# pavlidic/Binary-SpGEMM

Hardware: AMD Instinct MI355X
Metric: output nnz/sec (GNZ/s) (higher is better)
Workload: dtype int32; 1 GPU; R-MAT scale 22, edge factor 16, (a,b,c,d)=(0.30,0.25,0.25,0.20), seed 1, A*A; n=4194304, nnz_a=67108664, products=1336443900, nnz_c=1336366087, parallelism=row-shards x1 cut at equal work, B replicated, priming_steps=0, flow=auto, full=False

## Files before the change

### binary-spgemm_amd/csrc/context.hip

```cpp
#include "internal.hpp"

using namespace bsp;

thread_local char bspgemm_err_text[512] = "";

extern "C" const char *bspgemm_last_error(void) { return g_err; }

extern "C" const char *bspgemm_status_string(bspgemm_status s)
{
    switch (s) {
    case BSPGEMM_OK: return "ok";
    case BSPGEMM_ERR_INVALID: return "invalid argument";
    case BSPGEMM_ERR_ALLOC: return "allocation failed";
    case BSPGEMM_ERR_HIP: return "HIP runtime error";
    case BSPGEMM_ERR_NO_DEVICE: return "no gfx950 device (this library has no CPU fallback)";
    case BSPGEMM_ERR_OVERFLOW: return "result exceeds the int32 drop-in interface";
    case BSPGEMM_ERR_IO: return "file I/O error";
    case BSPGEMM_ERR_FORMAT: return "Matrix Market banner rejected";
    case BSPGEMM_ERR_SIZE: return "Matrix Market size line or entry rejected";
    case BSPGEMM_ERR_COMM: return "RCCL error";
    }
    return "unknown status";
}

// ... 99 lines not shown
    HIPCHK(hipGetDeviceProperties(&prop, device));
    if (strncmp(prop.gcnArchName, "gfx950", 6) != 0) {
        snprintf(g_err, sizeof g_err, "device %d is %s; libbspgemm carries gfx950 code only", device,
                 prop.gcnArchName);
        return BSPGEMM_ERR_NO_DEVICE;
    }
    bspgemm_context *ctx = new (std::nothrow) bspgemm_context();
    if (!ctx) return FAIL(BSPGEMM_ERR_ALLOC, "context");
    auto bail = [&](bspgemm_status st) { bspgemm_destroy(ctx); return st; };
    ctx->device = device;
    HIPCHK_B(hipSetDevice(device));
    HIPCHK_B(hipStreamCreateWithFlags(&ctx->stream, hipStreamNonBlocking));
    ctx->own_stream = true;
    HIPCHK_B(hipHostMalloc(reinterpret_cast<void **>(&ctx->h), sizeof(HostScalars), hipHostMallocDefault));
    HIPCHK_B(hipMalloc(reinterpret_cast<void **>(&ctx->d_prep), sizeof(PrepScalars)));
    HIPCHK_B(hipMalloc(reinterpret_cast<void **>(&ctx->d_small), sizeof(SmallScalars)));
    HIPCHK_B(hipMalloc(reinterpret_cast<void **>(&ctx->d_small_tiles), sizeof(SmallTiles)));
    HIPCHK_B(hipMalloc(reinterpret_cast<void **>(&ctx->d_err), 64));
    HIPCHK_B(hipMemset(ctx->d_err, 0, 64));
    HIPCHK_B(hipMalloc(reinterpret_cast<void **>(&ctx->bin_count), kNumBins * sizeof(int)));
    for (auto &sl : ctx->slots) {
        for (auto &e : sl.ev) HIPCHK_B(hipEventCreate(&e));
        for (auto &ph : sl.ev_cls) for (auto &c : ph) for (auto &e : c) HIPCHK_B(hipEventCreate(&e));
    }
    HIPCHK_B(hipStreamCreateWithFlags(&ctx->stream_b, hipStreamNonBlocking));
    HIPCHK_B(hipStreamCreateWithFlags(&ctx->stream_c, hipStreamNonBlocking));
    HIPCHK_B(hipEventCreateWithFlags(&ctx->ev_join, hipEventDisableTiming));
    for (auto &t : ctx->ev_tile) for (auto &e : t) HIPCHK_B(hipEventCreateWithFlags(&e, hipEventDisableTiming));
    ctx->cache_budget = prop.totalGlobalMem / 4;
    if (const char *e = getenv("BSPGEMM_FLOW"))
        ctx->flow = !strcmp(e, "exact") ? BSPGEMM_FLOW_EXACT : (!strcmp(e, "upper-bound") || !strcmp(e, "ub")) ? BSPGEMM_FLOW_UPPER_BOUND : BSPGEMM_FLOW_AUTO;
    if (const char *e = getenv("BSPGEMM_CLASS_TIMING")) ctx->class_timing = atoi(e) != 0;
    if (const char *e = getenv("BSPGEMM_CLASS_STREAMS")) { const int n = atoi(e); ctx->class_streams = n < 1 ? 1 : (n > 3 ? 3 : n); }
    ctx->check = getenv("BSPGEMM_CHECK") != nullptr;
    if (const char *e = getenv("BSPGEMM_RW_BLK")) ctx->rw_blk = atoi(e) ? 1 : 0;
    if (const char *e = getenv("BSPGEMM_SMALL")) ctx->small = atoi(e) ? 1 : 0;
    if (const char *e = getenv("BSPGEMM_PAD_ROWS")) { const int v = atoi(e); ctx->pad_rows = v < 0 ? -1 : (v ? 1 : 0); }
    ctx->debug_alloc = getenv("BSPGEMM_DEBUG_ALLOC") != nullptr;
    ctx->dropin_timing = getenv("BSPGEMM_DROPIN_TIMING") != nullptr;
    if (ctx->debug_alloc)
        fprintf(stderr, "[bspgemm] device %d: %s, %zu MiB, %d CUs; result cache budget %zu MiB\n", device,
                prop.gcnArchName, (size_t)(prop.totalGlobalMem >> 20), prop.multiProcessorCount, ctx->cache_budget >> 20);
    *out = ctx;
    return BSPGEMM_OK;
}

extern "C" void bspgemm_destroy(bspgemm_context *ctx)
{
    if (!ctx) return;
    hipSetDevice(ctx->device);
    if (ctx->stream) hipStreamSynchronize(ctx->stream);
    hipFree(ctx->F); hipFree(ctx->Fprefix); hipFree(ctx->partials);
    hipFree(ctx->cnt); hipFree(ctx->bin_tiles); hipFree(ctx->bin_count); hipFree(ctx->tmp); hipFree(ctx->tmpv);
    hipFree(ctx->rec); hipFree(ctx->recpre); hipFree(ctx->ab); hipFree(ctx->Fmask); hipFree(ctx->hpartials);
    hipFree(ctx->hub_rec); hipFree(ctx->hub_pre);
    if (ctx->h) hipHostFree(ctx->h);
    hipFree(ctx->d_prep);
    hipFree(ctx->d_err);
    hipFree(ctx->d_small);
    hipFree(ctx->d_small_tiles);
    hipFree(ctx->chunk_row);
    for (auto &sl : ctx->slots) {
        for (auto &e : sl.ev) if (e) hipEventDestroy(e);
        for (auto &ph : sl.ev_cls) for (auto &c : ph) for (auto &e : c) if (e) hipEventDestroy(e);
    }
    for (auto &c : ctx->cache) if (c.p) hipFree(c.p);
    if (ctx->stream_b) { hipStreamSynchronize(ctx->stream_b); hipStreamDestroy(ctx->stream_b); }
    if (ctx->stream_c) { hipStreamSynchronize(ctx->stream_c); hipStreamDestroy(ctx->stream_c); }
    if (ctx->ev_join) hipEventDestroy(ctx->ev_join);
    hipFree(ctx->stitch_partials);
    for (auto &t : ctx->ev_tile) for (auto &e : t) if (e) hipEventDestroy(e);
    if (ctx->own_stream && ctx->stream) hipStreamDestroy(ctx->stream);
    delete ctx;
}

extern "C" bspgemm_status bspgemm_set_stream(bspgemm_context *ctx, void *hip_stream)
{
    if (!ctx) return FAIL(BSPGEMM_ERR_INVALID, "ctx is NULL");
    if (bspgemm_status st = use_device(ctx)) return st;
    HIPCHK(hipStreamSynchronize(ctx->stream));
    if (hip_stream) {
        if (ctx->own_stream) hipStreamDestroy(ctx->stream);
        ctx->stream = static_cast<hipStream_t>(hip_stream);
        ctx->own_stream = false;
    } else if (!ctx->own_stream) {
        HIPCHK(hipStreamCreateWithFlags(&ctx->stream, hipStreamNonBlocking));
        ctx->own_stream = true;
    }
    return BSPGEMM_OK;
}

extern "C" bspgemm_status bspgemm_synchronize(bspgemm_context *ctx)
{
    if (!ctx) return FAIL(BSPGEMM_ERR_INVALID, "ctx is NULL");
    if (bspgemm_status st = use_device(ctx)) return st;
    HIPCHK(hipStreamSynchronize(ctx->stream));
    return BSPGEMM_OK;
}

extern "C" bspgemm_status bspgemm_matrix_upload(bspgemm_context *ctx, int rows, int cols,
                                                const int *row_ptr, const int *col_idx,
                                                bspgemm_matrix **out)
{
    if (!ctx || !out || !row_ptr || rows < 0 || cols < 0) return FAIL(BSPGEMM_ERR_INVALID, "matrix_upload");
    *out = nullptr;
    const long long base = row_ptr[0];
    const long long nnz = (long long)row_ptr[rows] - base;
// ... 74 lines not shown
    m->nnz_pad = 0;
    return BSPGEMM_OK;
}

extern "C" const char *bspgemm_build_info(void)
{
    return "libbspgemm: HIP kernels for gfx950 only; flows upper-bound (default), exact; small-product path; "
           "timing-only ablation switches: none (BSP_ABLATE=0); tuning constants are compile-time";
}

extern "C" int bspgemm_matrix_rows(const bspgemm_matrix *m) { return m ? m->rows : 0; }
extern "C" int bspgemm_matrix_cols(const bspgemm_matrix *m) { return m ? m->cols : 0; }
extern "C" int64_t bspgemm_matrix_nnz(const bspgemm_matrix *m) { return m ? m->nnz : 0; }

bspgemm_status ensure_rows(bspgemm_context *ctx, size_t rows)
{
    if (rows <= ctx->rows_cap) return BSPGEMM_OK;
    HIPCHK(hipStreamSynchronize(ctx->stream));
    hipFree(ctx->F); hipFree(ctx->Fprefix); hipFree(ctx->partials); hipFree(ctx->cnt); hipFree(ctx->bin_tiles);
    hipFree(ctx->rec); hipFree(ctx->recpre); hipFree(ctx->Fmask); hipFree(ctx->hpartials);
    ctx->F = ctx->Fprefix = ctx->partials = ctx->recpre = ctx->Fmask = ctx->hpartials = nullptr;
    ctx->cnt = ctx->bin_tiles = nullptr;
    ctx->rec = nullptr;
    ctx->rows_cap = 0;
    const size_t cap = rows + rows / 8 + 64;
    const size_t tiles = cap / 2048 + 2;
    HIPCHK(hipMalloc(reinterpret_cast<void **>(&ctx->F), cap * sizeof(long long)));
    HIPCHK(hipMalloc(reinterpret_cast<void **>(&ctx->Fmask), cap * sizeof(long long)));
    HIPCHK(hipMalloc(reinterpret_cast<void **>(&ctx->Fprefix), (cap + 1) * sizeof(long long)));
    HIPCHK(hipMalloc(reinterpret_cast<void **>(&ctx->partials), (tiles + 1) * sizeof(long long)));
    HIPCHK(hipMalloc(reinterpret_cast<void **>(&ctx->hpartials), (tiles + 1) * sizeof(long long)));
    HIPCHK(hipMalloc(reinterpret_cast<void **>(&ctx->cnt), cap * sizeof(int)));
    HIPCHK(hipMalloc(reinterpret_cast<void **>(&ctx->bin_tiles), (tiles + 1) * kNumBins * sizeof(int)));
    HIPCHK(hipMalloc(reinterpret_cast<void **>(&ctx->rec), cap * sizeof(RowRec)));
    HIPCHK(hipMalloc(reinterpret_cast<void **>(&ctx->recpre), cap * sizeof(long long)));
    if (!ctx->hub_rec) {
        HIPCHK(hipMalloc(reinterpret_cast<void **>(&ctx->hub_rec), kHeavySortMax * sizeof(RowRec)));
        HIPCHK(hipMalloc(reinterpret_cast<void **>(&ctx->hub_pre), kHeavySortMax * sizeof(long long)));
    }
    ctx->rows_cap = cap;
    return BSPGEMM_OK;
}

bspgemm_status ensure_ab(bspgemm_context *ctx, size_t pairs)
{
    if (pairs <= ctx->ab_cap) return BSPGEMM_OK;
    HIPCHK(hipStreamSynchronize(ctx->stream));
    hipFree(ctx->ab);
    ctx->ab = nullptr;
    ctx->ab_cap = 0;
    const size_t cap = pairs + pairs / 16 + 64;
    HIPCHK(hipMalloc(reinterpret_cast<void **>(&ctx->ab), cap * sizeof(int2)));
    ctx->ab_cap = cap;
    return BSPGEMM_OK;
}

bspgemm_status ensure_tmp(bspgemm_context *ctx, size_t ints)
{
    if (ints <= ctx->tmp_cap) return BSPGEMM_OK;
    HIPCHK(hipStreamSynchronize(ctx->stream));
    hipFree(ctx->tmp);
    ctx->tmp = nullptr;
    ctx->tmp_cap = 0;
    const size_t cap = ints + ints / 16 + 1024;
    hipError_t e = hipMalloc(reinterpret_cast<void **>(&ctx->tmp), cap * sizeof(int));
    if (e == hipErrorOutOfMemory) {
        for (auto &c : ctx->cache) if (c.p) { hipFree(c.p); c.p = nullptr; }
        (void)hipGetLastError();
        e = hipMalloc(reinterpret_cast<void **>(&ctx->tmp), cap * sizeof(int));
    }
    HIPCHK(e);
    ctx->tmp_cap = cap;
    return BSPGEMM_OK;
}

bspgemm_status ensure_tmpv(bspgemm_context *ctx, size_t ints)
{
    if (ints <= ctx->tmpv_cap) return BSPGEMM_OK;
    HIPCHK(hipStreamSynchronize(ctx->stream));
    hipFree(ctx->tmpv);
    ctx->tmpv = nullptr;
    ctx->tmpv_cap = 0;
    const size_t cap = ints + ints / 16 + 1024;
    hipError_t e = hipMalloc(reinterpret_cast<void **>(&ctx->tmpv), cap * sizeof(int));
    if (e == hipErrorOutOfMemory) {
        for (auto &c : ctx->cache) if (c.p) { hipFree(c.p); c.p = nullptr; }
        (void)hipGetLastError();
        e = hipMalloc(reinterpret_cast<void **>(&ctx->tmpv), cap * sizeof(int));
    }
    HIPCHK(e);
    ctx->tmpv_cap = cap;
    return BSPGEMM_OK;
}

bspgemm_status ensure_chunk_rows(bspgemm_context *ctx, size_t entries)
{
    if (entries <= ctx->chunk_cap) return BSPGEMM_OK;
    HIPCHK(hipStreamSynchronize(ctx->stream));
    hipFree(ctx->chunk_row);
    ctx->chunk_row = nullptr;
    ctx->chunk_cap = 0;
    const size_t cap = entries + entries / 16 + 64;
    HIPCHK(hipMalloc(reinterpret_cast<void **>(&ctx->chunk_row), cap * sizeof(int)));
    ctx->chunk_cap = cap;
    return BSPGEMM_OK;
}
// ... 234 lines not shown
```

### binary-spgemm_amd/csrc/internal.hpp

```cpp
#pragma once
#include "../../include/bspgemm.h"
#include "kernels.hpp"

#include <hip/hip_runtime.h>

#include <climits>
#include <cstdio>
#include <cstdlib>
#include <cstring>
#include <chrono>
#include <new>

extern thread_local char bspgemm_err_text[512];
#define g_err bspgemm_err_text

static inline bspgemm_status fail(bspgemm_status st, const char *what, const char *file, int line)
{
    snprintf(g_err, sizeof g_err, "%s (%s:%d)", what, file, line);
    return st;
}
#define FAIL(st, what) fail((st), (what), __FILE__, __LINE__)
#define HIPCHK(call)                                                                       \
    do {                                                                                   \
        hipError_t e_ = (call);                                                            \
// ... 13 lines not shown
        }                                                                                  \
    } while (0)

using bsp::kNumBins;
using bsp::PrepScalars;
using bsp::RowRec;
struct HostScalars {
    long long totalF;
    long long nnzC;
    int bin_count[kNumBins];
    int a_lo, a_hi;
    long long products;
    long long heavy_total;
    PrepScalars prep;
    unsigned err;
    bsp::SmallScalars small;
};

struct bspgemm_context {
    int device = 0;
    hipStream_t stream = nullptr;
    bool own_stream = false;
    hipStream_t stream_b = nullptr;
    hipStream_t stream_c = nullptr;
    hipEvent_t ev_tile[2][3] = {};
    hipEvent_t ev_join = nullptr;
    struct StatSlot {
        hipEvent_t ev[5] = {};
        hipEvent_t ev_cls[2][kNumBins][2] = {};
        int R = 0;
        bool cls_timed = false;
        int mid_cap = 0, rank_cap = 0;
        HostScalars h = {};
        long long products = 0, nnz_c = 0;
        int cls_n[2][kNumBins] = {};
        bool used = false;
        int flow = 0, prepass_kernel = 0, class_streams = 0;
        bool small = false, checked = false, padded = false;
    };
    static constexpr int kStatSlots = 16;
    StatSlot slots[kStatSlots];
    int slot_head = 0;
    long long *stitch_partials = nullptr;
    size_t stitch_partials_cap = 0;
    size_t rows_cap = 0;
    long long *F = nullptr, *Fprefix = nullptr, *partials = nullptr, *recpre = nullptr, *Fmask = nullptr;
    long long *hpartials = nullptr;
    RowRec *hub_rec = nullptr;
    long long *hub_pre = nullptr;
    int *cnt = nullptr, *bin_tiles = nullptr, *bin_count = nullptr;
    RowRec *rec = nullptr;
    size_t ab_cap = 0;
    int2 *ab = nullptr;
    size_t tmp_cap = 0;
    int *tmp = nullptr;
    size_t tmpv_cap = 0;
    int *tmpv = nullptr;
    PrepScalars *d_prep = nullptr;
    bsp::SmallScalars *d_small = nullptr;
    bsp::SmallTiles *d_small_tiles = nullptr;
    unsigned *d_err = nullptr;
    int *chunk_row = nullptr;
    size_t chunk_cap = 0;
    HostScalars *h = nullptr;
    struct CachedBuf { void *p; size_t bytes; };
    CachedBuf cache[8] = {};
    size_t cache_budget = 0;
    int flow = BSPGEMM_FLOW_AUTO;
    bool class_timing = false;
    int class_streams = 2;
    bool check = false;
    int rw_blk = -1;
    int pad_rows = 0;
    int small = -1;
    bool debug_alloc = false;
    bool dropin_timing = false;
};

extern "C" int bspgemm_par_max_plus_one(const int *idx, long long n);
extern "C" void bspgemm_par_prefault(void *p, size_t bytes);
extern "C" long long bspgemm_par_output_bound(const int *Acol, const int *Arow, int r0, int r1, const int *Brow, int brows, long long cap);

struct bspgemm_matrix {
    bspgemm_context *ctx;
    int rows, cols;
    long long nnz;
    int *d_row_ptr, *d_col_idx;
    bool owned;
    mutable unsigned char *d_deg8 = nullptr;
    mutable int *d_blk8 = nullptr;
    mutable int blk8_state = 0;
    mutable int *d_col_pad = nullptr;
    mutable int *d_row_ptr_pad = nullptr;
    mutable int2 *d_ext = nullptr;
    mutable int pad_state = 0;
    mutable long long nnz_pad = 0;
    const int *gather_col() const { return pad_state == 1 ? d_col_pad : d_col_idx; }
    long long gather_nnz() const { return pad_state == 1 ? nnz_pad : nnz; }
};

bspgemm_status ensure_deg8(const bspgemm_matrix *m);
bspgemm_status ensure_blk8(const bspgemm_matrix *m);
bspgemm_status ensure_pad(const bspgemm_matrix *m);

struct bspgemm_result {
    bspgemm_context *ctx;
    int rows;
    long long nnz;
    long long *d_row_ptr;
    int *d_col_idx;
    long long col_cap;
    int *d_values = nullptr;
};

bspgemm_status use_device(bspgemm_context *ctx);

bspgemm_status ensure_rows(bspgemm_context *ctx, size_t rows);
bspgemm_status ensure_ab(bspgemm_context *ctx, size_t pairs);
bspgemm_status ensure_tmp(bspgemm_context *ctx, size_t ints);
bspgemm_status ensure_tmpv(bspgemm_context *ctx, size_t ints);
bspgemm_status ensure_chunk_rows(bspgemm_context *ctx, size_t entries);
bool result_cached(const bspgemm_context *ctx, size_t bytes);
hipError_t result_alloc(bspgemm_context *ctx, void **out, size_t bytes);
void result_release(bspgemm_context *ctx, void *p, size_t bytes);
static inline size_t result_bytes_rowptr(int rows) { return ((size_t)rows + 1) * sizeof(long long); }
static inline size_t result_bytes_colidx(long long nnz) { return ((size_t)nnz + 4) * sizeof(int); }

int dropin_fail(const char *fn, bspgemm_status st);
```

### binary-spgemm_amd/csrc/kernels.hpp

```cpp
#pragma once
#include <hip/hip_runtime.h>
#include <stdint.h>
#include <stdlib.h>

namespace bsp {

enum class MaskMode { None, Keep, Drop, Insert, Count };

constexpr int kWaveBins = 16;
constexpr int kNumBins = kWaveBins + 4;
constexpr int kRankBin = kWaveBins + 1;
constexpr int kMidBin = kWaveBins + 2;
constexpr int kDenseBin = kWaveBins + 3;
constexpr int kRankCap = 6144;
int rank_cap_for_cols(long long cols);
constexpr int kMaxBins = 20;
constexpr int kWaveChunks[kWaveBins + 1] = {0, 1, 2, 3, 4, 5, 6, 7, 8, 10, 12, 14, 16, 20, 24, 28, 32};
constexpr int kMaxWaveCap = 64 * kWaveChunks[kWaveBins];
constexpr int kMidCap = 524288;
inline int mid_cap_for_cols(long long cols)
{
    const long long passes = (cols + (1ll << 18) - 1) >> 18;
    if (passes <= 1) return kMidCap;
    const long long c = kMidCap / passes;
    return c < kMaxWaveCap ? kMaxWaveCap : (int)c;
}
constexpr int kRowsPerWave = 16;

constexpr int kWaveTopWords = 256;

inline int levels_for_cols(int64_t cols)
{
    for (int L = 1; L < 5; L++)
        if (cols <= ((int64_t)kWaveTopWords << (5 * L))) return L;
    return 5;
}

constexpr int kWaveTopWordsWide = 512;
inline int wave_levels_for_cols(int64_t cols)
{
    const int L = levels_for_cols(cols);
    if (L == 4 && cols <= ((int64_t)kWaveTopWordsWide << 15)) return 3;
    return L;
}

struct RowRec {
    int row;
    int a0;
    int alen;
    int f;
};

void launch_row_work(const int *Arow, const int *Acol, const int *Brow, const int *Bblk8, const int *Bpad, const int2 *Bext,
                     int row_begin, int row_end, long long *F, int2 *ab, hipStream_t s);
void launch_blk8(const int *row_ptr, const int *start_ptr, int n, int *blk, unsigned long long *clamped_nnz, hipStream_t s);
void launch_pad_lengths(const int *row_ptr, int n, int *plen, hipStream_t s);
void launch_pad_copy(const int *row_ptr, const int *col_idx, const int *pad_ptr, int n, int *col_pad, int2 *ext, hipStream_t s);

void launch_deg8(const int *row_ptr, int n, unsigned char *deg8, hipStream_t s);
void launch_row_products(const int *Arow, const int *Acol, const int *Brow, const unsigned char *Bdeg8,
                         int row_begin, int row_end, long long *F, hipStream_t s);

struct PrepScalars {
    long long totalF;
    long long heavy_total;
    long long products;
    int a_lo, a_hi;
    int bin_count[kNumBins];
    unsigned long long max_f;
};
void launch_scan_and_bin(const long long *F, int n, int row_begin, const int *Arow, long long *prefix,
                         long long *partials, int *bin_tiles, int *bin_count, RowRec *rec,
                         long long *recpre, int *cnt, int heavy_cols, long long *hpartials, int mid_cap, int rank_cap, int bound_cols,
                         hipStream_t s, PrepScalars *scal = nullptr, const long long *true_F = nullptr);

constexpr int kCompactGran = 4096;
inline size_t compact_chunk_rows(long long max_out) { return (size_t)((max_out + kCompactGran - 1) / kCompactGran) + 2; }
void launch_scan_counts(const int *cnt, int n, long long *prefix, long long *partials,
                        const long long *base, hipStream_t s, int *chunk_row = nullptr);

constexpr unsigned kErrCapacity = 1u;
constexpr unsigned kErrStaleTable = 2u;
hipError_t launch_wave_rows(int bin, int levels, const int2 *ab, const int *Bcol, int cols,
                            const RowRec *rec, const long long *recpre, const long long *row_ptr, int nrows,
                            int row_begin, int *tmp, int *cnt, unsigned *err, MaskMode mode, const int *Frow, const int *Fcol,
                            hipStream_t s, bool count_only = false);
void launch_check_tables(const int *row_ptr, int rows, const unsigned char *deg8, const int *blk8, const int *pad_ptr, unsigned *err,
                         hipStream_t s);

void launch_place_heavy(const int *tmp, const RowRec *rec, const long long *recpre, int nrows,
                        const long long *row_ptr, int row_begin, int *col_idx, hipStream_t s);

hipError_t launch_dense_rows(int bin, const int2 *ab, const int *Bcol, long long nnzB, int cols,
                             const RowRec *rec, const long long *recpre, int nrows, int row_begin,
                             int *tmp, int *cnt, MaskMode mode, const int *Frow, const int *Fcol, hipStream_t s,
                             int *vals = nullptr);

constexpr int kHeavySortMax = 8192;
void launch_order_heavy(const RowRec *rec, const long long *recpre, int n, RowRec *rec_out, long long *pre_out, hipStream_t s);

bool wave_masked_supported(int cols);
void launch_wave_masked(int bin, const int2 *ab, const int *Bcol, int cols, const int *Frow, const int *Fcol,
                        const RowRec *rec, const long long *recpre, int nrows, int row_begin,
                        int *tmp, int *cnt, int *vals, hipStream_t s);
hipError_t launch_class(int bin, const int2 *ab, const int *Bcol, long long nnzB, int cols, const RowRec *rec,
                        const long long *recpre, int nrows, int row_begin, int *tmp, int *cnt, unsigned *err, MaskMode mode,
                        const int *Frow, const int *Fcol, hipStream_t s, bool count_only = false, int *vals = nullptr);
// ... 36 lines not shown
```

### binary-spgemm_amd/csrc/multiply.hip

```cpp
#include "internal.hpp"

using namespace bsp;

static bspgemm_status check_operands(bspgemm_context *ctx, const bspgemm_matrix *A, const bspgemm_matrix *B,
                                     int row_begin, int row_end)
{
    if (!ctx || !A || !B) return FAIL(BSPGEMM_ERR_INVALID, "NULL operand");
    if (A->ctx != ctx || B->ctx != ctx) return FAIL(BSPGEMM_ERR_INVALID, "operand belongs to another context");
    if (row_begin < 0 || row_end < row_begin || row_end > A->rows) return FAIL(BSPGEMM_ERR_INVALID, "row range");
    if (B->rows < A->cols) return FAIL(BSPGEMM_ERR_INVALID, "B has fewer rows than A has columns");
    return BSPGEMM_OK;
}


static void class_order(const int *bin_count, long long total_products, int *order, int *lane)
{
    int light[kWaveBins];
    for (int k = 0; k < kWaveBins; k++) light[k] = k + 1;
    const long long heavy_lower_bound = ((long long)bin_count[kRankBin] + bin_count[kMidBin] + bin_count[kDenseBin]) * kMaxWaveCap;
    if (heavy_lower_bound * 8 < total_products) {
        long long key[kNumBins] = {};
        for (int b = 1; b <= kWaveBins; b++) key[b] = (long long)bin_count[b] * kWaveChunks[b];
        for (int a = 1; a < kWaveBins; a++)
            for (int c = a; c > 0 && key[light[c]] > key[light[c - 1]]; c--) {
// ... 31 lines not shown
    bspgemm_context::StatSlot &slot = ctx->slots[ctx->slot_head];
    slot.used = false;
    slot.flow = flow;
    slot.class_streams = small ? 1 : ctx->class_streams;
    slot.small = small;
    slot.checked = !small && ctx->check;
    return slot;
}

static void close_slot(bspgemm_context *ctx, int R, const HostScalars *h, long long products, long long nnz_c,
                       const int (*cls_n)[kNumBins], int mid_cap, int rank_cap = 0)
{
    bspgemm_context::StatSlot &sl = ctx->slots[ctx->slot_head];
    sl.R = R;
    sl.cls_timed = ctx->class_timing;
    sl.mid_cap = mid_cap;
    sl.rank_cap = rank_cap;
    sl.h = *h;
    sl.products = products;
    sl.nnz_c = nnz_c;
    memcpy(sl.cls_n, cls_n, sizeof sl.cls_n);
    sl.used = true;
}

static bspgemm_status drop_result(bspgemm_result *C, bspgemm_status st)
{
    const bspgemm_context *ctx = C->ctx;
    hipStreamSynchronize(ctx->stream); hipStreamSynchronize(ctx->stream_b); hipStreamSynchronize(ctx->stream_c);
    bspgemm_result_free(C);
    return st;
}

static hipError_t alloc_col_idx(bspgemm_context *ctx, bspgemm_result *C, long long cap)
{
    if (hipError_t e = result_alloc(ctx, reinterpret_cast<void **>(&C->d_col_idx), result_bytes_colidx(cap))) return e;
    C->col_cap = cap;
    return hipSuccess;
}
static long long col_cap_for(long long bound, long long nnz_c) { return (bound - nnz_c <= nnz_c / 50 + 4096) ? bound : nnz_c; }

static bspgemm_status start_flow(bspgemm_context *ctx, const bspgemm_matrix *A, const bspgemm_matrix *B,
                                 const bspgemm_matrix *Fm, int row_begin, int row_end, int flow, bspgemm_result **out,
                                 bspgemm_result **Cp)
{
    if (!out) return FAIL(BSPGEMM_ERR_INVALID, "result pointer is NULL");
    *out = nullptr;
    if (bspgemm_status st = check_operands(ctx, A, B, row_begin, row_end)) return st;
    if (Fm && (Fm->ctx != ctx || Fm->rows < row_end)) return FAIL(BSPGEMM_ERR_INVALID, "mask has fewer rows than A / wrong context");
    if (bspgemm_status st = use_device(ctx)) return st;
    const int R = row_end - row_begin;
    hipStream_t s = ctx->stream;
    if (bspgemm_status st = ensure_rows(ctx, (size_t)R + 1)) return st;
    if (bspgemm_status st = ensure_ab(ctx, (size_t)A->nnz + 1)) return st;

    bspgemm_result *C = new (std::nothrow) bspgemm_result{ctx, R, 0, nullptr, nullptr, 0};
    if (!C) return FAIL(BSPGEMM_ERR_ALLOC, "result");
    auto bail = [&](bspgemm_status st) { return drop_result(C, st); };
    bspgemm_context::StatSlot &slot = open_slot(ctx, flow, false);
    HIPCHK_B(hipEventRecord(slot.ev[0], s));
    HIPCHK_B(result_alloc(ctx, reinterpret_cast<void **>(&C->d_row_ptr), result_bytes_rowptr(R)));
    if (bspgemm_status st = ensure_pad(B)) return bail(st);
    if (bspgemm_status st = ensure_blk8(B)) return bail(st);
    if (ctx->check) {
        HIPCHK_B(hipMemsetAsync(ctx->d_err, 0, sizeof(unsigned), s));
        launch_check_tables(B->d_row_ptr, B->rows, B->d_deg8, B->blk8_state == 1 ? B->d_blk8 : nullptr,
                            B->pad_state == 1 ? B->d_row_ptr_pad : nullptr, ctx->d_err, s);
    }
    slot.prepass_kernel = B->blk8_state == 1 ? 1 : 0;
    slot.padded = B->pad_state == 1;
    launch_row_work(A->d_row_ptr, A->d_col_idx, B->d_row_ptr, B->blk8_state == 1 ? B->d_blk8 : nullptr,
                    B->pad_state == 1 ? B->d_row_ptr_pad : nullptr, B->pad_state == 1 ? B->d_ext : nullptr, row_begin, row_end,
                    ctx->F, ctx->ab, s);
    *Cp = C;
    return BSPGEMM_OK;
}

template <class Launch>
static bspgemm_status class_phase(bspgemm_context *ctx, int phase, long long products, int *cls_n, bool heavy_on_third,
                                  Launch launch)
{
    const int *bin_count = ctx->h->bin_count;
    hipStream_t lanes[3] = {ctx->stream, ctx->stream_b, ctx->stream_c};
    const int nlanes = ctx->class_streams;
    hipEvent_t *tile = ctx->ev_tile[phase];
    hipEvent_t (*ev_cls)[2] = ctx->slots[ctx->slot_head].ev_cls[phase];
    size_t bin_start[kNumBins + 1] = {0, 0};
    for (int b = 1; b < kNumBins; b++) bin_start[b + 1] = bin_start[b] + (size_t)bin_count[b];
    int order[kNumBins], lane_of[kNumBins];
    class_order(bin_count, products, order, lane_of);

    HIPCHK(hipEventRecord(tile[0], lanes[0]));
    for (int l = 1; l < 3; l++)
        if (l < nlanes || (l == 2 && heavy_on_third)) HIPCHK(hipStreamWaitEvent(lanes[l], tile[0], 0));
    for (int pos = 1; pos < kNumBins; pos++) {
        const int b = order[pos];
        const int n = bin_count[b];
        cls_n[b] = n;
        if (n <= 0) continue;
        hipStream_t sx = heavy_on_third && b > kWaveBins ? lanes[2] : lanes[lane_of[pos] % nlanes];
        if (ctx->class_timing) HIPCHK(hipEventRecord(ev_cls[b][0], sx));
        HIPCHK(launch(b, n, ctx->rec + bin_start[b], ctx->recpre + bin_start[b], sx));
        if (ctx->class_timing) HIPCHK(hipEventRecord(ev_cls[b][1], sx));
    }
    HIPCHK(hipGetLastError());
    for (int l = 1; l < nlanes; l++) {
        HIPCHK(hipEventRecord(tile[l], lanes[l]));
        HIPCHK(hipStreamWaitEvent(lanes[0], tile[l], 0));
    }
    return BSPGEMM_OK;
}

static bspgemm_status finish_flow(bspgemm_context *ctx, bspgemm_result *C, const bspgemm_matrix *B, long long products,
                                  int rank_cap, const int (*cls_n)[kNumBins], bspgemm_result **out)
{
    auto bail = [&](bspgemm_status st) { return drop_result(C, st); };
    hipStream_t s = ctx->stream;
    HostScalars *h = ctx->h;
    HIPCHK_B(hipEventRecord(ctx->slots[ctx->slot_head].ev[4], s));
    if (ctx->check) HIPCHK_B(hipMemcpyAsync(&h->err, ctx->d_err, sizeof(unsigned), hipMemcpyDeviceToHost, s));
    HIPCHK_B(hipStreamSynchronize(s));
    if (ctx->check && h->err)
        return bail(FAIL(BSPGEMM_ERR_INVALID, (h->err & kErrStaleTable)
            ? "operand B was rewritten in place: its derived tables do not match its row_ptr (call bspgemm_matrix_invalidate)"
            : "a row gathered more products than its capacity class holds (operand changed during the multiply?)"));
    C->nnz = h->nnzC;
// ... 464 lines not shown
```

### binary-spgemm_amd/csrc/prepass.hip

```cpp
#include "kernels.hpp"
#include "wave.hpp"

namespace bsp {

struct __attribute__((packed, aligned(4))) Int2U { int x, y; };

constexpr int kLongRow = 256;
constexpr int kRowWorkUnroll = 4;
template <typename Sweep>
__device__ __forceinline__ long long rows_of_a_wave(int a0, int a1, int sub, Sweep &&sweep)
{
    const int lane = threadIdx.x & 63;
    long long long_sum = 0;
#pragma unroll
    for (int q = 0; q < 8; q++) {
        const int qa0 = __builtin_amdgcn_readlane(a0, q * 8), qa1 = __builtin_amdgcn_readlane(a1, q * 8);
        if (qa1 - qa0 > kLongRow) {
            long long t = sweep((long long)qa0 + lane, (long long)qa1, 64);
#pragma unroll
            for (int d = 1; d < 64; d <<= 1) t += __shfl_xor(t, d, 64);
            if (lane == q * 8) long_sum = t;
        }
    }
    const bool is_long = a1 - a0 > kLongRow;
// ... 35 lines not shown
                }
            }
#pragma unroll
            for (int u = 0; u < U; u++)
                if (j[u] >= 0) {
                    const int len = pr[u].y - pr[u].x;
                    ab[jj + stride * u] = make_int2(pr[u].x, len);
                    sum += (long long)len;
                }
        }
        return sum;
    };
    const long long sum = rows_of_a_wave(a0, a1, sub, sweep);
    if (r < nrows && sub == 0) F[r] = sum;
}

struct __attribute__((packed, aligned(4))) Blk8 { int base; unsigned lo, hi; };

__global__ __launch_bounds__(256) void k_blk8(const int *__restrict__ row_ptr, const int *__restrict__ start_ptr, int n,
                                              int *__restrict__ blk, unsigned long long *__restrict__ clamped_nnz)
{
    const int b = blockIdx.x * blockDim.x + threadIdx.x;
    if (b * 8 >= n) return;
    const int r0 = b * 8;
    unsigned lo = 0u, hi = 0u;
    long long clamped = 0;
    int prev = row_ptr[r0];
    const int base = start_ptr[r0];
#pragma unroll
    for (int k = 0; k < 8; k++) {
        int d = 0;
        if (r0 + k < n) {
            const int nx = row_ptr[r0 + k + 1];
            d = nx - prev;
            prev = nx;
        }
        const unsigned byte = (unsigned)(d < 255 ? d : 255);
        if (d >= 255) clamped += d;
        if (k < 4) lo |= byte << (8 * k); else hi |= byte << (8 * (k - 4));
    }
    if (clamped > 0) atomicAdd(clamped_nnz, (unsigned long long)clamped);
    blk[3 * b] = base;
    blk[3 * b + 1] = (int)lo;
    blk[3 * b + 2] = (int)hi;
}
void launch_blk8(const int *row_ptr, const int *start_ptr, int n, int *blk, unsigned long long *clamped_nnz, hipStream_t s)
{
    if (n <= 0) return;
    const int nb = (n + 7) / 8;
    hipLaunchKernelGGL(k_blk8, dim3((nb + 255) / 256), dim3(256), 0, s, row_ptr, start_ptr ? start_ptr : row_ptr, n, blk, clamped_nnz);
}

template <bool PAD>
__global__ __launch_bounds__(256) void k_row_work_blk(const int *__restrict__ Arow,
                                                      const int *__restrict__ Acol,
                                                      const int *__restrict__ Brow,
                                                      const int *__restrict__ Bblk,
                                                      const int *__restrict__ Bpad,
                                                      int row_begin, int nrows,
                                                      long long *__restrict__ F,
                                                      int2 *__restrict__ ab)
{
    const long long gid = (long long)blockIdx.x * blockDim.x + threadIdx.x;
    const int r = (int)(gid >> 3);
    const int sub = (int)(gid & 7);
    int a0 = 0, a1 = 0;
    if (r < nrows) { a0 = Arow[row_begin + r]; a1 = Arow[row_begin + r + 1]; }
    constexpr int U = kRowWorkUnroll;
    auto sweep = [&](long long first, long long end, int stride) {
        long long sum = 0;
        for (long long jj = first; jj < end; jj += (long long)stride * U) {
            int j[U];
#pragma unroll
            for (int u = 0; u < U; u++) j[u] = (jj + stride * u < end) ? Acol[jj + stride * u] : -1;
            Blk8 w[U];
#pragma unroll
            for (int u = 0; u < U; u++) {
                w[u].base = 0; w[u].lo = w[u].hi = 0u;
                if (j[u] >= 0) w[u] = *reinterpret_cast<const Blk8 *>(Bblk + 3 * (j[u] >> 3));
            }
            int start[U], len[U];
            bool sat[U];
#pragma unroll
            for (int u = 0; u < U; u++) {
                const int k = j[u] & 7;
                const u64 d = ((u64)w[u].hi << 32) | (u64)w[u].lo;
                const u64 below = d & ((1ull << (8 * k)) - 1ull);
                const u64 upto = (k == 7) ? d : (d & ((1ull << (8 * k + 8)) - 1ull));
                const u64 v = ~upto;
                sat[u] = j[u] >= 0 && ((v - 0x0101010101010101ull) & ~v & 0x8080808080808080ull) != 0ull;
                if (PAD) {
                    const u64 m0f = 0x0f0f0f0f0f0f0f0full, m01 = 0x0101010101010101ull;
                    const u64 units = ((below >> 4) & m0f) + ((((below & m0f) + m0f) >> 4) & m01);
                    start[u] = w[u].base + 16 * ((int)__builtin_amdgcn_sad_u8((unsigned)units, 0u, 0u)
                                                 + (int)__builtin_amdgcn_sad_u8((unsigned)(units >> 32), 0u, 0u));
                } else {
                    start[u] = w[u].base + (int)__builtin_amdgcn_sad_u8((unsigned)below, 0u, 0u)
                               + (int)__builtin_amdgcn_sad_u8((unsigned)(below >> 32), 0u, 0u);
                }
                len[u] = (int)((d >> (8 * k)) & 255ull);
            }
            Int2U pr[U];
            int ps[U];
#pragma unroll
            for (int u = 0; u < U; u++) {
                pr[u].x = pr[u].y = 0;
                ps[u] = 0;
                if (sat[u]) {
                    pr[u] = *reinterpret_cast<const Int2U *>(Brow + j[u]);
                    if (PAD) ps[u] = Bpad[j[u]];
                }
            }
#pragma unroll
            for (int u = 0; u < U; u++)
                if (j[u] >= 0) {
                    if (sat[u]) { start[u] = PAD ? ps[u] : pr[u].x; len[u] = pr[u].y - pr[u].x; }
                    ab[jj + stride * u] = make_int2(start[u], len[u]);
                    sum += (long long)len[u];
                }
        }
        return sum;
    };
    const long long sum = rows_of_a_wave(a0, a1, sub, sweep);
    if (r < nrows && sub == 0) F[r] = sum;
}

void launch_row_work(const int *Arow, const int *Acol, const int *Brow, const int *Bblk8, const int *Bpad, const int2 *Bext,
                     int row_begin, int row_end, long long *F, int2 *ab, hipStream_t s)
{
    const int nrows = row_end - row_begin;
    if (nrows <= 0) return;
    const long long threads = (long long)nrows * 8;
    const int grid = (int)((threads + 255) / 256);
    if (Bblk8 && Bpad)
        hipLaunchKernelGGL(k_row_work_blk<true>, dim3(grid), dim3(256), 0, s, Arow, Acol, Brow, Bblk8, Bpad, row_begin, nrows, F, ab);
    else if (Bblk8)
        hipLaunchKernelGGL(k_row_work_blk<false>, dim3(grid), dim3(256), 0, s, Arow, Acol, Brow, Bblk8, nullptr, row_begin, nrows, F, ab);
    else if (Bext)
        hipLaunchKernelGGL(k_row_work<true>, dim3(grid), dim3(256), 0, s, Arow, Acol, Brow, Bext, row_begin, nrows, F, ab);
    else
        hipLaunchKernelGGL(k_row_work<false>, dim3(grid), dim3(256), 0, s, Arow, Acol, Brow, nullptr, row_begin, nrows, F, ab);
}

__global__ __launch_bounds__(256) void k_pad_lengths(const int *__restrict__ row_ptr, int n, int *__restrict__ plen)
{
    const int i = blockIdx.x * blockDim.x + threadIdx.x;
    if (i < n) plen[i] = ((row_ptr[i + 1] - row_ptr[i]) + 15) & ~15;
}
void launch_pad_lengths(const int *row_ptr, int n, int *plen, hipStream_t s)
{
    if (n <= 0) return;
    hipLaunchKernelGGL(k_pad_lengths, dim3((n + 255) / 256), dim3(256), 0, s, row_ptr, n, plen);
}
__global__ __launch_bounds__(256) void k_pad_copy(const int *__restrict__ row_ptr, const int *__restrict__ col_idx,
                                                  const int *__restrict__ pad_ptr, int n, int *__restrict__ col_pad,
                                                  int2 *__restrict__ ext)
{
    const long long gid = (long long)blockIdx.x * blockDim.x + threadIdx.x;
    const int r = (int)(gid >> 4), sub = (int)(gid & 15);
    if (r >= n) return;
    const int s0 = row_ptr[r], len = row_ptr[r + 1] - s0, d0 = pad_ptr[r];
    const int plen = (len + 15) & ~15;
    for (int t = sub; t < plen; t += 16) col_pad[d0 + t] = col_idx[s0 + (t < len ? t : len - 1)];
    if (sub == 0 && ext) ext[r] = make_int2(d0, len);
}
void launch_pad_copy(const int *row_ptr, const int *col_idx, const int *pad_ptr, int n, int *col_pad, int2 *ext, hipStream_t s)
{
    if (n <= 0) return;
    const long long threads = (long long)n * 16;
    hipLaunchKernelGGL(k_pad_copy, dim3((unsigned)((threads + 255) / 256)), dim3(256), 0, s, row_ptr, col_idx, pad_ptr, n, col_pad, ext);
}

__global__ __launch_bounds__(256) void k_deg8(const int *__restrict__ row_ptr, int n, unsigned char *__restrict__ deg8)
{
    const int i = blockIdx.x * blockDim.x + threadIdx.x;
    if (i < n) {
        const int d = row_ptr[i + 1] - row_ptr[i];
        deg8[i] = (unsigned char)(d < 255 ? d : 255);
    }
}
void launch_deg8(const int *row_ptr, int n, unsigned char *deg8, hipStream_t s)
{
    if (n <= 0) return;
    hipLaunchKernelGGL(k_deg8, dim3((n + 255) / 256), dim3(256), 0, s, row_ptr, n, deg8);
}

__global__ __launch_bounds__(256) void k_row_products(const int *__restrict__ Arow, const int *__restrict__ Acol,
                                                      const int *__restrict__ Brow,
                                                      const unsigned char *__restrict__ Bdeg8,
                                                      int row_begin, int nrows, long long *__restrict__ F)
{
// ... 386 lines not shown
```

Before: 215.7 GNZ/s.

## Replace row-parallel blk8 row-work kernel with merge-path flat tiling over nonzeros

The blk8 row-work pass, which computes per-A-nonzero B extents and per-row product counts F, now splits work into fixed tiles of 4096 merged (row + nonzero) items instead of assigning 8 threads per A row. A small k_tile_rows kernel first maps each tile to its starting row. The flat kernel then does coalesced loads, scans the lengths in shared memory, and writes F directly for rows wholly inside a tile or via atomicAdd for rows that span tiles. This targets load imbalance from skewed R-MAT row lengths, at the cost of an extra launch, atomics on boundary rows, and heavier shared-memory use.

```diff
diff --git a/binary-spgemm_amd/csrc/context.hip b/binary-spgemm_amd/csrc/context.hip
--- a/binary-spgemm_amd/csrc/context.hip
+++ b/binary-spgemm_amd/csrc/context.hip
@@ -175,7 +175,7 @@
     if (ctx->stream) hipStreamSynchronize(ctx->stream);
     hipFree(ctx->F); hipFree(ctx->Fprefix); hipFree(ctx->partials);
     hipFree(ctx->cnt); hipFree(ctx->bin_tiles); hipFree(ctx->bin_count); hipFree(ctx->tmp); hipFree(ctx->tmpv);
-    hipFree(ctx->rec); hipFree(ctx->recpre); hipFree(ctx->ab); hipFree(ctx->Fmask); hipFree(ctx->hpartials);
+    hipFree(ctx->rec); hipFree(ctx->recpre); hipFree(ctx->ab); hipFree(ctx->tile_row); hipFree(ctx->Fmask); hipFree(ctx->hpartials);
     hipFree(ctx->hub_rec); hipFree(ctx->hub_pre);
     if (ctx->h) hipHostFree(ctx->h);
     hipFree(ctx->d_prep);
@@ -356,6 +356,20 @@
     const size_t cap = pairs + pairs / 16 + 64;
     HIPCHK(hipMalloc(reinterpret_cast<void **>(&ctx->ab), cap * sizeof(int2)));
     ctx->ab_cap = cap;
+    return BSPGEMM_OK;
+}
+
+bspgemm_status ensure_tile_rows(bspgemm_context *ctx, size_t items)
+{
+    const size_t need = items / kRowWorkTile + 2;
+    if (need <= ctx->tile_row_cap) return BSPGEMM_OK;
+    HIPCHK(hipStreamSynchronize(ctx->stream));
+    hipFree(ctx->tile_row);
+    ctx->tile_row = nullptr;
+    ctx->tile_row_cap = 0;
+    const size_t cap = need + need / 16 + 64;
+    HIPCHK(hipMalloc(reinterpret_cast<void **>(&ctx->tile_row), cap * sizeof(int)));
+    ctx->tile_row_cap = cap;
     return BSPGEMM_OK;
 }
 
diff --git a/binary-spgemm_amd/csrc/internal.hpp b/binary-spgemm_amd/csrc/internal.hpp
--- a/binary-spgemm_amd/csrc/internal.hpp
+++ b/binary-spgemm_amd/csrc/internal.hpp
@@ -89,6 +89,8 @@
     RowRec *rec = nullptr;
     size_t ab_cap = 0;
     int2 *ab = nullptr;
+    size_t tile_row_cap = 0;
+    int *tile_row = nullptr;
     size_t tmp_cap = 0;
     int *tmp = nullptr;
     size_t tmpv_cap = 0;
@@ -154,6 +156,7 @@
 
 bspgemm_status ensure_rows(bspgemm_context *ctx, size_t rows);
 bspgemm_status ensure_ab(bspgemm_context *ctx, size_t pairs);
+bspgemm_status ensure_tile_rows(bspgemm_context *ctx, size_t items);
 bspgemm_status ensure_tmp(bspgemm_context *ctx, size_t ints);
 bspgemm_status ensure_tmpv(bspgemm_context *ctx, size_t ints);
 bspgemm_status ensure_chunk_rows(bspgemm_context *ctx, size_t entries);
diff --git a/binary-spgemm_amd/csrc/kernels.hpp b/binary-spgemm_amd/csrc/kernels.hpp
--- a/binary-spgemm_amd/csrc/kernels.hpp
+++ b/binary-spgemm_amd/csrc/kernels.hpp
@@ -51,8 +51,9 @@
     int f;
 };
 
+constexpr int kRowWorkTile = 4096;
 void launch_row_work(const int *Arow, const int *Acol, const int *Brow, const int *Bblk8, const int *Bpad, const int2 *Bext,
-                     int row_begin, int row_end, long long *F, int2 *ab, hipStream_t s);
+                     int row_begin, int row_end, long long nnz_bound, int *tile_row, long long *F, int2 *ab, hipStream_t s);
 void launch_blk8(const int *row_ptr, const int *start_ptr, int n, int *blk, unsigned long long *clamped_nnz, hipStream_t s);
 void launch_pad_lengths(const int *row_ptr, int n, int *plen, hipStream_t s);
 void launch_pad_copy(const int *row_ptr, const int *col_idx, const int *pad_ptr, int n, int *col_pad, int2 *ext, hipStream_t s);
diff --git a/binary-spgemm_amd/csrc/multiply.hip b/binary-spgemm_amd/csrc/multiply.hip
--- a/binary-spgemm_amd/csrc/multiply.hip
+++ b/binary-spgemm_amd/csrc/multiply.hip
@@ -107,6 +107,7 @@
     hipStream_t s = ctx->stream;
     if (bspgemm_status st = ensure_rows(ctx, (size_t)R + 1)) return st;
     if (bspgemm_status st = ensure_ab(ctx, (size_t)A->nnz + 1)) return st;
+    if (bspgemm_status st = ensure_tile_rows(ctx, (size_t)A->nnz + (size_t)R)) return st;
 
     bspgemm_result *C = new (std::nothrow) bspgemm_result{ctx, R, 0, nullptr, nullptr, 0};
     if (!C) return FAIL(BSPGEMM_ERR_ALLOC, "result");
@@ -125,7 +126,7 @@
     slot.padded = B->pad_state == 1;
     launch_row_work(A->d_row_ptr, A->d_col_idx, B->d_row_ptr, B->blk8_state == 1 ? B->d_blk8 : nullptr,
                     B->pad_state == 1 ? B->d_row_ptr_pad : nullptr, B->pad_state == 1 ? B->d_ext : nullptr, row_begin, row_end,
-                    ctx->F, ctx->ab, s);
+                    A->nnz, ctx->tile_row, ctx->F, ctx->ab, s);
     *Cp = C;
     return BSPGEMM_OK;
 }
diff --git a/binary-spgemm_amd/csrc/prepass.hip b/binary-spgemm_amd/csrc/prepass.hip
--- a/binary-spgemm_amd/csrc/prepass.hip
+++ b/binary-spgemm_amd/csrc/prepass.hip
@@ -111,91 +111,171 @@
 }
 
 template <bool PAD>
-__global__ __launch_bounds__(256) void k_row_work_blk(const int *__restrict__ Arow,
-                                                      const int *__restrict__ Acol,
-                                                      const int *__restrict__ Brow,
-                                                      const int *__restrict__ Bblk,
-                                                      const int *__restrict__ Bpad,
-                                                      int row_begin, int nrows,
-                                                      long long *__restrict__ F,
-                                                      int2 *__restrict__ ab)
-{
-    const long long gid = (long long)blockIdx.x * blockDim.x + threadIdx.x;
-    const int r = (int)(gid >> 3);
-    const int sub = (int)(gid & 7);
-    int a0 = 0, a1 = 0;
-    if (r < nrows) { a0 = Arow[row_begin + r]; a1 = Arow[row_begin + r + 1]; }
-    constexpr int U = kRowWorkUnroll;
-    auto sweep = [&](long long first, long long end, int stride) {
-        long long sum = 0;
-        for (long long jj = first; jj < end; jj += (long long)stride * U) {
-            int j[U];
-#pragma unroll
-            for (int u = 0; u < U; u++) j[u] = (jj + stride * u < end) ? Acol[jj + stride * u] : -1;
-            Blk8 w[U];
-#pragma unroll
-            for (int u = 0; u < U; u++) {
-                w[u].base = 0; w[u].lo = w[u].hi = 0u;
-                if (j[u] >= 0) w[u] = *reinterpret_cast<const Blk8 *>(Bblk + 3 * (j[u] >> 3));
-            }
-            int start[U], len[U];
-            bool sat[U];
-#pragma unroll
-            for (int u = 0; u < U; u++) {
-                const int k = j[u] & 7;
-                const u64 d = ((u64)w[u].hi << 32) | (u64)w[u].lo;
-                const u64 below = d & ((1ull << (8 * k)) - 1ull);
-                const u64 upto = (k == 7) ? d : (d & ((1ull << (8 * k + 8)) - 1ull));
-                const u64 v = ~upto;
-                sat[u] = j[u] >= 0 && ((v - 0x0101010101010101ull) & ~v & 0x8080808080808080ull) != 0ull;
-                if (PAD) {
-                    const u64 m0f = 0x0f0f0f0f0f0f0f0full, m01 = 0x0101010101010101ull;
-                    const u64 units = ((below >> 4) & m0f) + ((((below & m0f) + m0f) >> 4) & m01);
-                    start[u] = w[u].base + 16 * ((int)__builtin_amdgcn_sad_u8((unsigned)units, 0u, 0u)
-                                                 + (int)__builtin_amdgcn_sad_u8((unsigned)(units >> 32), 0u, 0u));
-                } else {
-                    start[u] = w[u].base + (int)__builtin_amdgcn_sad_u8((unsigned)below, 0u, 0u)
-                               + (int)__builtin_amdgcn_sad_u8((unsigned)(below >> 32), 0u, 0u);
-                }
-                len[u] = (int)((d >> (8 * k)) & 255ull);
-            }
-            Int2U pr[U];
-            int ps[U];
-#pragma unroll
-            for (int u = 0; u < U; u++) {
-                pr[u].x = pr[u].y = 0;
-                ps[u] = 0;
-                if (sat[u]) {
-                    pr[u] = *reinterpret_cast<const Int2U *>(Brow + j[u]);
-                    if (PAD) ps[u] = Bpad[j[u]];
-                }
-            }
-#pragma unroll
-            for (int u = 0; u < U; u++)
-                if (j[u] >= 0) {
-                    if (sat[u]) { start[u] = PAD ? ps[u] : pr[u].x; len[u] = pr[u].y - pr[u].x; }
-                    ab[jj + stride * u] = make_int2(start[u], len[u]);
-                    sum += (long long)len[u];
-                }
-        }
-        return sum;
-    };
-    const long long sum = rows_of_a_wave(a0, a1, sub, sweep);
-    if (r < nrows && sub == 0) F[r] = sum;
+__device__ __forceinline__ void blk8_extent(const Blk8 &w, int j, int &start, int &len, bool &sat)
+{
+    const int k = j & 7;
+    const u64 d = ((u64)w.hi << 32) | (u64)w.lo;
+    const u64 below = d & ((1ull << (8 * k)) - 1ull);
+    const u64 upto = (k == 7) ? d : (d & ((1ull << (8 * k + 8)) - 1ull));
+    const u64 v = ~upto;
+    sat = ((v - 0x0101010101010101ull) & ~v & 0x8080808080808080ull) != 0ull;
+    if (PAD) {
+        const u64 m0f = 0x0f0f0f0f0f0f0f0full, m01 = 0x0101010101010101ull;
+        const u64 units = ((below >> 4) & m0f) + ((((below & m0f) + m0f) >> 4) & m01);
+        start = w.base + 16 * ((int)__builtin_amdgcn_sad_u8((unsigned)units, 0u, 0u)
+                               + (int)__builtin_amdgcn_sad_u8((unsigned)(units >> 32), 0u, 0u));
+    } else {
+        start = w.base + (int)__builtin_amdgcn_sad_u8((unsigned)below, 0u, 0u)
+                + (int)__builtin_amdgcn_sad_u8((unsigned)(below >> 32), 0u, 0u);
+    }
+    len = (int)((d >> (8 * k)) & 255ull);
+}
+
+constexpr int kFlatTile = kRowWorkTile;
+constexpr int kFlatK = kFlatTile / 256;
+
+__global__ __launch_bounds__(256) void k_tile_rows(const int *__restrict__ Arow, int row_begin, int nrows,
+                                                   int *__restrict__ tile_row, long long *__restrict__ F)
+{
+    const int r = blockIdx.x * blockDim.x + threadIdx.x;
+    if (r >= nrows) return;
+    const long long lo = Arow[row_begin];
+    const long long m0 = Arow[row_begin + r] - lo + r, m1 = Arow[row_begin + r + 1] - lo + r;
+    for (long long t = (m0 + kFlatTile - 1) / kFlatTile; t * kFlatTile <= m1; t++) tile_row[t] = r;
+    if (m0 / kFlatTile != m1 / kFlatTile) F[r] = 0;
+}
+
+template <bool PAD>
+__global__ __launch_bounds__(256) void k_row_work_flat(const int *__restrict__ Arow,
+                                                       const int *__restrict__ Acol,
+                                                       const int *__restrict__ Brow,
+                                                       const int *__restrict__ Bblk,
+                                                       const int *__restrict__ Bpad,
+                                                       int row_begin, int nrows,
+                                                       const int *__restrict__ tile_row,
+                                                       long long *__restrict__ F,
+                                                       int2 *__restrict__ ab)
+{
+    constexpr int K = kFlatK, NB = kFlatTile, RV = kFlatK + 1;
+    constexpr int LSTRIDE = K + 4;
+    __shared__ __attribute__((aligned(16))) long long P[NB + NB / 16 + 1];
+    __shared__ long long wsum[4];
+    static_assert(256 * LSTRIDE * sizeof(int) <= sizeof(P), "staged lengths do not fit the prefix array");
+    int *L = reinterpret_cast<int *>(P);
+    auto pidx = [](int q) { return q + (q >> 4); };
+
+    const int tid = threadIdx.x;
+    const int *rp = Arow + row_begin;
+    const long long lo = rp[0], nnz = rp[nrows] - lo, total = nnz + nrows;
+    const long long d0 = (long long)blockIdx.x * NB;
+    if (d0 >= total) return;
+    const bool last = d0 + NB >= total;
+    const long long d1 = last ? total : d0 + NB;
+    const int rb = tile_row[blockIdx.x];
+    const int rl = last ? nrows - 1 : tile_row[blockIdx.x + 1];
+    const long long j0 = d0 - rb, j1 = last ? nnz : d1 - rl;
+    const int n = (int)(j1 - j0);
+    const long long g0 = lo + j0;
+    int fa0 = 0, fa1 = 0;
+    if (rb + tid <= rl) { fa0 = rp[rb + tid]; fa1 = rp[rb + tid + 1]; }
+
+    int j[K];
+#pragma unroll
+    for (int k = 0; k < K; k++) j[k] = tid + 256 * k < n ? Acol[g0 + tid + 256 * k] : -1;
+    Blk8 w[K];
+#pragma unroll
+    for (int k = 0; k < K; k++) {
+        w[k].base = 0; w[k].lo = w[k].hi = 0u;
+        if (j[k] >= 0) w[k] = *reinterpret_cast<const Blk8 *>(Bblk + 3 * (j[k] >> 3));
+    }
+    int start[K], len[K];
+    bool sat[K];
+#pragma unroll
+    for (int k = 0; k < K; k++) {
+        blk8_extent<PAD>(w[k], j[k], start[k], len[k], sat[k]);
+        sat[k] = sat[k] && j[k] >= 0;
+    }
+    Int2U pr[K];
+    int ps[K];
+#pragma unroll
+    for (int k = 0; k < K; k++) {
+        pr[k].x = pr[k].y = 0;
+        ps[k] = 0;
+        if (sat[k]) {
+            pr[k] = *reinterpret_cast<const Int2U *>(Brow + j[k]);
+            if (PAD) ps[k] = Bpad[j[k]];
+        }
+    }
+#pragma unroll
+    for (int k = 0; k < K; k++) {
+        const int p = tid + 256 * k;
+        if (sat[k]) { start[k] = PAD ? ps[k] : pr[k].x; len[k] = pr[k].y - pr[k].x; }
+        if (j[k] < 0) len[k] = 0;
+        else ab[g0 + p] = make_int2(start[k], len[k]);
+        L[p + 4 * (p / K)] = len[k];
+    }
+    __syncthreads();
+
+    int mine[K];
+#pragma unroll
+    for (int i = 0; i < K; i += 4) {
+        const int4 v = *reinterpret_cast<const int4 *>(L + LSTRIDE * tid + i);
+        mine[i] = v.x; mine[i + 1] = v.y; mine[i + 2] = v.z; mine[i + 3] = v.w;
+    }
+    long long tot = 0;
+#pragma unroll
+    for (int i = 0; i < K; i++) tot += mine[i];
+    const long long inc = wave_incl_scan64(tot);
+    const int lane = tid & 63, wv = tid >> 6;
+    if (lane == 63) wsum[wv] = inc;
+    __syncthreads();
+    long long off = inc - tot;
+    for (int k = 0; k < wv; k++) off += wsum[k];
+#pragma unroll
+    for (int i = 0; i < K; i++) {
+        off += mine[i];
+        P[pidx(K * tid + i + 1)] = off;
+    }
+    if (tid == 0) P[0] = 0;
+    int ra0[RV], ra1[RV];
+    ra0[0] = fa0;
+    ra1[0] = fa1;
+#pragma unroll
+    for (int i = 1; i < RV; i++)
+        if (rb + tid + 256 * i <= rl) { ra0[i] = rp[rb + tid + 256 * i]; ra1[i] = rp[rb + tid + 256 * i + 1]; }
+    __syncthreads();
+
+#pragma unroll
+    for (int i = 0; i < RV; i++) {
+        const int r = rb + tid + 256 * i;
+        if (r > rl) break;
+        const long long a0 = ra0[i] - lo, a1 = ra1[i] - lo;
+        const long long s = a0 > j0 ? a0 : j0, e = a1 < j1 ? a1 : j1;
+        const long long v = e > s ? P[pidx((int)(e - j0))] - P[pidx((int)(s - j0))] : 0;
+        if (a0 + r >= d0 && a1 + r < d1) F[r] = v;
+        else if (v != 0) atomicAdd(reinterpret_cast<unsigned long long *>(F + r), (unsigned long long)v);
+    }
 }
 
 void launch_row_work(const int *Arow, const int *Acol, const int *Brow, const int *Bblk8, const int *Bpad, const int2 *Bext,
-                     int row_begin, int row_end, long long *F, int2 *ab, hipStream_t s)
+                     int row_begin, int row_end, long long nnz_bound, int *tile_row, long long *F, int2 *ab, hipStream_t s)
 {
     const int nrows = row_end - row_begin;
     if (nrows <= 0) return;
+    if (Bblk8) {
+        hipLaunchKernelGGL(k_tile_rows, dim3((nrows + 255) / 256), dim3(256), 0, s, Arow, row_begin, nrows, tile_row, F);
+        const int tiles = (int)((nnz_bound + nrows + kFlatTile - 1) / kFlatTile);
+        if (Bpad)
+            hipLaunchKernelGGL(k_row_work_flat<true>, dim3(tiles), dim3(256), 0, s, Arow, Acol, Brow, Bblk8, Bpad, row_begin, nrows,
+                               tile_row, F, ab);
+        else
+            hipLaunchKernelGGL(k_row_work_flat<false>, dim3(tiles), dim3(256), 0, s, Arow, Acol, Brow, Bblk8, nullptr, row_begin,
+                               nrows, tile_row, F, ab);
+        return;
+    }
     const long long threads = (long long)nrows * 8;
     const int grid = (int)((threads + 255) / 256);
-    if (Bblk8 && Bpad)
-        hipLaunchKernelGGL(k_row_work_blk<true>, dim3(grid), dim3(256), 0, s, Arow, Acol, Brow, Bblk8, Bpad, row_begin, nrows, F, ab);
-    else if (Bblk8)
-        hipLaunchKernelGGL(k_row_work_blk<false>, dim3(grid), dim3(256), 0, s, Arow, Acol, Brow, Bblk8, nullptr, row_begin, nrows, F, ab);
-    else if (Bext)
+    if (Bext)
         hipLaunchKernelGGL(k_row_work<true>, dim3(grid), dim3(256), 0, s, Arow, Acol, Brow, Bext, row_begin, nrows, F, ab);
     else
         hipLaunchKernelGGL(k_row_work<false>, dim3(grid), dim3(256), 0, s, Arow, Acol, Brow, nullptr, row_begin, nrows, F, ab);
```

Measured after the change: 225.9 GNZ/s (median of 6 runs). 1.05x the previous value.
